# tanmayrainanda/ishara

Measured on AMD Instinct MI355X. Metric: landmark-frames/sec training (B=256,T=384,d=256), higher is better.
Workload: dtype bf16; 1 GPU; configs[1]: get_model(dim=256, 2 squeeze + 2 conformer blocks, kernel_sizes=[11,5,3]) CTC train step (fwd+CTC+bwd+RAdam/Lookahead, dropout on); batch_per_gpu=256, global_batch=256, frames=384, features=224, params=7577784, parallelism=dp1, ranks_seen=1

## Files before the change

ishara_amd/csrc/gemm_as.hip:

```cpp
#include <cstdio>
#include <map>
#include <string>
#include <type_traits>
#include "common.h"
#include "kernels.h"

#ifdef AS_F16
typedef f16 as_t;
typedef f16x8 as_v8;
#define AS_MFMA(b, a, acc) __builtin_amdgcn_mfma_f32_16x16x32_f16(b, a, acc, 0, 0, 0)
#define AS_DT DT_F16
#define AS_NAME(x) x##_f16
#else
typedef bf16 as_t;
typedef bf16x8 as_v8;
#define AS_MFMA(b, a, acc) __builtin_amdgcn_mfma_f32_16x16x32_bf16(b, a, acc, 0, 0, 0)
#define AS_DT DT_BF16
#define AS_NAME(x) x
#endif

extern int g_force_regstage;
bool gemm_nt_as_applicable(int dtC, int M, int N, int K, int ldb, const EpiArgs& ea);

#define AS_NS 32
#define AS_SMALL_M 1536
#define AS_MID_M_K512 32768
#define AS_MAXN 1024

typedef __attribute__((ext_vector_type(4))) uint32_t as_u32x4;

template <int N> DEVI void as_wait_vm() { asm volatile("s_waitcnt vmcnt(%0)" ::"n"(N) : "memory"); }

DEVI int as_swz(int r) { return (r & 3) | (((r >> 3) & 1) << 2); }

template <int GW, typename T> DEVI void as_st(T* p, const float (&v)[GW]) {
    if constexpr (GW == 8) store8(p, v); else store4(p, v);
}
template <int GW, typename T> DEVI void as_st_nt(T* p, const float (&v)[GW], bool nt = true) {
    if constexpr (GW == 8 && is_16b_t<T>::value) {
        as_v8 t;
#pragma unroll
        for (int i = 0; i < 8; ++i) t[i] = (as_t)v[i];
        if (nt) __builtin_nontemporal_store(t, reinterpret_cast<as_v8*>(p)); else *reinterpret_cast<as_v8*>(p) = t;
    } else as_st<GW>(p, v);
}
DEVI void as_st_pk(as_t* p, const as_v8& t, bool nt) {
    if (nt) __builtin_nontemporal_store(t, reinterpret_cast<as_v8*>(p)); else *reinterpret_cast<as_v8*>(p) = t;
}
template <typename TC, int GW> DEVI void as_unpack(const as_u32x4& r, float (&v)[GW]) {
    if constexpr (GW == 8 && std::is_same<TC, f16>::value) {
        const f16x8 h = __builtin_bit_cast(f16x8, r);
#pragma unroll
        for (int e = 0; e < 8; ++e) v[e] = (float)h[e];
    } else if constexpr (GW == 8) {
#pragma unroll
        for (int h = 0; h < 4; ++h) { v[2 * h] = __uint_as_float(r[h] << 16); v[2 * h + 1] = __uint_as_float(r[h] & 0xffff0000u); }
    } else {
#pragma unroll
        for (int h = 0; h < 4; ++h) v[h] = __uint_as_float(r[h]);
    }
}

enum { AS_RESID = 1, AS_DACT = 2, AS_ACT = 4, AS_DROP = 8, AS_ROWSCALE = 16, AS_PREOUT = 32, AS_QKV = 64, AS_ADDTAB = 128, AS_ALL = 255 };
template <int MASK, int F> DEVI bool as_on(bool runtime) {
    if constexpr ((MASK & F) == 0) return false;
    else if constexpr (MASK == AS_ALL) return runtime;
    else return true;
}

template <typename TC, int KT, int MASK, int RT, int DBG, int PRO, int NW = 4, int CS = 1>
DEVI void as_pass(const as_t* __restrict__ A, const as_t* __restrict__ Bt, TC* __restrict__ C, int M, int N, int ldb, const EpiArgs& ea,
                  char* smem, const float* bias_s, int m_base) {
    constexpr int RB = KT * 64;
    constexpr int NS = AS_NS;
    constexpr int SUB = NS * RB;
    constexpr int STAGE = SUB * CS;
    constexpr int R = CS > 1 ? 2 : (KT <= 8 ? 3 : 2);
    constexpr int K = KT * 32;
    constexpr int NI = STAGE / 1024;
    constexpr int DPW = (NI + NW - 1) / NW;
    constexpr bool PAIR = is_16b_t<TC>::value;
    constexpr int GW = PAIR ? 8 : 4;
    constexpr int NG = NS / (4 * GW);
    constexpr int SPS = RT * NG;
    constexpr bool COUNTED = (MASK & (AS_RESID | AS_DACT | AS_ADDTAB | AS_QKV)) == 0;
    constexpr int OPS = SPS * ((MASK & AS_PREOUT) ? 2 : 1);
    constexpr bool HOLDABLE = PAIR && std::is_same<TC, as_t>::value && MASK != AS_ALL && (MASK & AS_QKV) == 0;
    const bool hold = HOLDABLE && (ea.as_flags & 1) && !ea.n_valid;
    const bool nt_side = (ea.as_flags & 2) != 0;

    const int dbg = DBG ? ea.dbg : 0;
    const int tid = threadIdx.x, lane = tid & 63;
    const int wid = __builtin_amdgcn_readfirstlane(tid >> 6);
    const int c = lane & 15, g = lane >> 4;
    const int mw = m_base + wid * 16 * RT;
    const bool full = m_base + NW * 16 * RT <= M;
    const int nsteps = N / NS / (int)gridDim.y;
    const int nbase = (int)blockIdx.y * nsteps * NS;
    const int dmodel = ea.H * ea.dh;
    const bool f_resid = as_on<MASK, AS_RESID>(ea.resid != nullptr), f_dact = as_on<MASK, AS_DACT>(ea.dact != DACT_NONE);
    const bool f_act = as_on<MASK, AS_ACT>(ea.act != ACT_NONE), f_drop = as_on<MASK, AS_DROP>(ea.drop.thr != 0);
    const bool f_rowscale = as_on<MASK, AS_ROWSCALE>(ea.rowscale != nullptr), f_preout = as_on<MASK, AS_PREOUT>(ea.pre_out != nullptr);
    const bool f_qkv = as_on<MASK, AS_QKV>(ea.mode == EPI_QKV), f_addtab = as_on<MASK, AS_ADDTAB>(ea.addtab != nullptr);

    const as_t* bsrc[DPW];
#pragma unroll
    for (int t = 0; t < DPW; ++t) {
        const int o = ((wid * DPW + t) % NI) * 1024 + lane * 16;
        const int r = o / RB, p = (o % RB) >> 4;
        bsrc[t] = Bt + (size_t)(nbase + r) * ldb + ((p ^ as_swz(r)) << 3);
    }
    const size_t bstep = (size_t)NS * CS * ldb;
    auto issue = [&](int slot) {
#pragma unroll
        for (int t = 0; t < DPW; ++t) {
            __builtin_amdgcn_global_load_lds((const __attribute__((address_space(1))) void*)bsrc[t],
                                             (__attribute__((address_space(3))) void*)(smem + slot + ((wid * DPW + t) % NI) * 1024), 16, 0, 0);
            bsrc[t] += bstep;
        }
    };
    const int nstages = (nsteps + CS - 1) / CS;
#pragma unroll
    for (int st = 0; st < R - 1; ++st)
        if (st < nstages && !(dbg & 8)) issue(st * STAGE);

    as_v8 a[RT][KT];
    int mrow[RT];
#pragma unroll
    for (int i = 0; i < RT; ++i) {
        mrow[i] = min(mw + 16 * i + c, M - 1);
        const as_v8* p = reinterpret_cast<const as_v8*>(A + (size_t)mrow[i] * K + g * 8);
#pragma unroll
        for (int kt = 0; kt < KT; ++kt) a[i][kt] = p[kt * 4];
    }

    if constexpr (PRO != 0) {
        float* cs = reinterpret_cast<float*>(smem + (R - 1) * STAGE);
        const int bsm = min(m_base, M - 1) / ea.T;
        const float* c0 = PRO == 1 ? ea.ln_gamma : ea.pa_P + (size_t)bsm * K;
        const float* c1 = PRO == 1 ? ea.ln_beta : ea.pa_Q + (size_t)bsm * K;
        for (int x = tid; x < K; x += NW * 64) { cs[x] = c0[x]; cs[K + x] = c1[x]; }
        __syncthreads();
        auto unpack = [&](const as_v8& f, float (&v)[8]) {
            as_u32x4 t = __builtin_bit_cast(as_u32x4, f);
            asm volatile("" : "+v"(t));
            as_unpack<as_t, 8>(t, v);
        };
        float mean[RT], rstd[RT];
#pragma unroll
        for (int i = 0; i < RT; ++i) { mean[i] = 0.f; rstd[i] = 1.f; }
        if constexpr (PRO == 1) {
#pragma unroll
            for (int i = 0; i < RT; ++i) {
                float s = 0.f;
#pragma unroll
                for (int kt = 0; kt < KT; ++kt) {
                    float v[8];
                    unpack(a[i][kt], v);
#pragma unroll
                    for (int e = 0; e < 8; ++e) s += v[e];
                }
                s += __shfl_xor(s, 16, 64); s += __shfl_xor(s, 32, 64);
                mean[i] = s * (1.f / K);
                float q = 0.f;
#pragma unroll
                for (int kt = 0; kt < KT; ++kt) {
                    float v[8];
                    unpack(a[i][kt], v);
#pragma unroll
                    for (int e = 0; e < 8; ++e) { const float dlt = v[e] - mean[i]; q += dlt * dlt; }
                }
                q += __shfl_xor(q, 16, 64); q += __shfl_xor(q, 32, 64);
                rstd[i] = rsqrtf(q * (1.f / K) + ea.ln_eps);
                const int m = mw + 16 * i + c;
                if (g == 0 && m < M && ea.ln_mean && blockIdx.y == 0) { ea.ln_mean[m] = mean[i]; ea.ln_rstd[m] = rstd[i]; }
            }
        }
#pragma unroll
        for (int kt = 0; kt < KT; ++kt) {
            float wv[8], bv[8];
            {
                const float* cp = cs + 32 * kt + 8 * g;
                asm volatile("" : "+v"(cp));
                const f32x4 w0 = *reinterpret_cast<const f32x4*>(cp), w1 = *reinterpret_cast<const f32x4*>(cp + 4);
                const f32x4 b0 = *reinterpret_cast<const f32x4*>(cp + K), b1 = *reinterpret_cast<const f32x4*>(cp + K + 4);
#pragma unroll
                for (int e = 0; e < 4; ++e) { wv[e] = w0[e]; wv[4 + e] = w1[e]; bv[e] = b0[e]; bv[4 + e] = b1[e]; }
            }
#pragma unroll
            for (int i = 0; i < RT; ++i) {
                float v[8];
                unpack(a[i][kt], v);
                as_v8 t;
#pragma unroll
                for (int e = 0; e < 8; ++e) t[e] = (as_t)(PRO == 1 ? (v[e] - mean[i]) * rstd[i] * wv[e] + bv[e] : v[e] * wv[e] + bv[e]);
                a[i][kt] = t;
            }
        }
        __syncthreads();
    }

    const int frow = PAIR ? 8 * (c >> 2) + (c & 3) : c;
    const int sx = g ^ as_swz(frow);
    const int off_e = frow * RB + ((sx & 3) << 4) + ((sx >> 2) << 6);
    const int off_o = frow * RB + ((sx & 3) << 4) + (((sx >> 2) ^ 1) << 6);
    constexpr int JSTRIDE = (PAIR ? 4 : 16) * RB;

    float rsc[RT];
    uint32_t rk[RT];
    int bsamp[RT];
#pragma unroll
    for (int i = 0; i < RT; ++i) {
        const int m = mw + 16 * i + c;
        rsc[i] = 1.f; rk[i] = 0u; bsamp[i] = 0;
        if (f_rowscale || f_qkv) bsamp[i] = mrow[i] / ea.T;
        if (f_rowscale) rsc[i] = ea.rowscale[bsamp[i]];
        if (f_drop) rk[i] = rng_row_key(ea.drop.key, (uint32_t)m);
    }

    size_t eoff[RT];
#pragma unroll
    for (int i = 0; i < RT; ++i) eoff[i] = (size_t)mrow[i] * (ea.ldc ? ea.ldc : N) + GW * g;
    const TC* resid = reinterpret_cast<const TC*>(ea.resid);
    const TC* aux = reinterpret_cast<const TC*>(ea.aux);

#pragma unroll
    for (int i = 0; i < RT; ++i) {
#pragma unroll
        for (int kt = 0; kt < KT; ++kt) {
            as_u32x4 t = __builtin_bit_cast(as_u32x4, a[i][kt]);
            asm volatile("" : "+v"(t));
            a[i][kt] = __builtin_bit_cast(as_v8, t);
        }
        asm volatile("" : "+v"(rsc[i]));
    }

    as_v8 held[RT], held_pre[RT];
#pragma unroll
    for (int i = 0; i < RT; ++i) { held[i] = as_v8{}; held_pre[i] = as_v8{}; }
    int slot = 0;
    for (int s = 0; s < nsteps; ++s) {
        const int sub = CS > 1 ? (s & (CS - 1)) : 0;
        const bool sync = CS == 1 || sub == 0;
        const int sg = CS > 1 ? s / CS : s;
        if (sync) {
            if constexpr (CS > 1) {
                constexpr bool CCOUNT = MASK != AS_ALL && (MASK & AS_QKV) == 0;
                if (CCOUNT && full && !ea.n_valid && sg >= 1) as_wait_vm<CS * OPS>(); else as_wait_vm<0>();
            } else if constexpr (COUNTED) {
                if (full && !ea.n_valid && s >= R - 1 && s + R - 2 < nsteps) {
                    if (!hold) as_wait_vm<(R - 2) * DPW + (R - 1) * OPS>();
                    else if constexpr (R == 3) as_wait_vm<DPW + 2 * OPS>();
                    else { if (s & 1) as_wait_vm<0>(); else as_wait_vm<2 * OPS>(); }
                } else as_wait_vm<0>();
            } else {
                if (s + R - 2 < nsteps) as_wait_vm<(R - 2) * DPW>(); else as_wait_vm<0>();
            }
            asm volatile("s_waitcnt lgkmcnt(0)" ::: "memory");
            __builtin_amdgcn_s_barrier();
        }
        const int n0 = nbase + s * NS;
        as_u32x4 rs[RT][NG], au[RT][NG];
        if (f_resid) {
#pragma unroll
            for (int i = 0; i < RT; ++i)
#pragma unroll
                for (int q = 0; q < NG; ++q) rs[i][q] = *reinterpret_cast<const as_u32x4*>(resid + eoff[i] + n0 + 4 * GW * q);
        }
        if (f_dact) {
#pragma unroll
            for (int i = 0; i < RT; ++i)
#pragma unroll
                for (int q = 0; q < NG; ++q) au[i][q] = __builtin_nontemporal_load(reinterpret_cast<const as_u32x4*>(aux + eoff[i] + n0 + 4 * GW * q));
        }
        if (sync && sg + R - 1 < nstages && !(dbg & 8)) issue(slot == 0 ? (R - 1) * STAGE : slot - STAGE);
        f32x4 acc[2][RT];
#pragma unroll
        for (int j = 0; j < 2; ++j)
#pragma unroll
            for (int i = 0; i < RT; ++i) acc[j][i] = f32x4{0.f, 0.f, 0.f, 0.f};
        const char* st = smem + slot + sub * SUB;
        if (!(dbg & 6)) {
#pragma unroll
            for (int kt = 0; kt < KT; ++kt) {
#pragma unroll
                for (int j = 0; j < 2; ++j) {
                    const as_v8 b = *reinterpret_cast<const as_v8*>(st + ((kt & 1) ? off_o : off_e) + (kt >> 1) * 128 + j * JSTRIDE);
#pragma unroll
                    for (int i = 0; i < RT; ++i) acc[j][i] = AS_MFMA(b, a[i][kt], acc[j][i]);
                }
            }
        } else if (!(dbg & 4)) {
#pragma unroll
            for (int kt = 0; kt < KT; ++kt)
#pragma unroll
                for (int j = 0; j < 2; ++j) {
                    const f32x4 b = *reinterpret_cast<const f32x4*>(st + ((kt & 1) ? off_o : off_e) + (kt >> 1) * 128 + j * JSTRIDE);
                    acc[j][0] += b;
                }
        } else if (!(dbg & 2)) {
            const as_v8 b = a[0][0];
#pragma unroll
            for (int kt = 0; kt < KT; ++kt)
#pragma unroll
                for (int j = 0; j < 2; ++j)
#pragma unroll
                    for (int i = 0; i < RT; ++i) acc[j][i] = AS_MFMA(b, a[i][kt], acc[j][i]);
        } else {
#pragma unroll
            for (int i = 0; i < RT; ++i) acc[0][i][0] = (float)a[i][0][0] + (float)a[i][KT - 1][7];
        }
        if (dbg & 1) { if (acc[0][0][0] == 123.456f) C[0] = from_f<TC>(acc[1][RT - 1][2]); if (CS == 1 || sub == CS - 1) slot = slot == (R - 1) * STAGE ? 0 : slot + STAGE; continue; }
#pragma unroll
        for (int q = 0; q < NG; ++q) {
            const int n = n0 + 4 * GW * q + GW * g;
            if (ea.n_valid && n >= ea.n_valid) continue;
            float bias[GW];
#pragma unroll
            for (int h = 0; h < GW / 4; ++h) {
                const f32x4 bv = *reinterpret_cast<const f32x4*>(bias_s + n + 4 * h);
#pragma unroll
                for (int e = 0; e < 4; ++e) bias[4 * h + e] = bv[e];
            }
#pragma unroll
            for (int i = 0; i < RT; ++i) {
                const int m = mw + 16 * i + c;
                if (!full && m >= M) continue;
                const size_t off = eoff[i] + n0 + 4 * GW * q;
                float v[GW];
                const float bsc = (f_rowscale && ea.rowscale_bias) ? rsc[i] : 1.f;
                if constexpr (PAIR) {
#pragma unroll
                    for (int e = 0; e < 4; ++e) { v[e] = acc[0][i][e] + bias[e] * bsc; v[4 + e] = acc[1][i][e] + bias[4 + e] * bsc; }
                } else {
#pragma unroll
                    for (int e = 0; e < 4; ++e) v[e] = acc[q][i][e] + bias[e] * bsc;
                }
                if (f_addtab) {
                    const float* tp = ea.addtab + (size_t)(m % ea.tab_period) * N + n;
#pragma unroll
                    for (int h = 0; h < GW / 4; ++h) {
                        float t4[4];
                        load4(tp + 4 * h, t4);
#pragma unroll
                        for (int e = 0; e < 4; ++e) v[4 * h + e] += t4[e];
                    }
                }
                if (f_preout) {
                    if constexpr (HOLDABLE) {
                        if (hold) {
                            as_v8 t;
#pragma unroll
                            for (int e = 0; e < 8; ++e) t[e] = (as_t)v[e];
                            as_t* pp = reinterpret_cast<as_t*>(ea.pre_out) + off;
                            if (s & 1) { as_st_pk(pp - NS, held_pre[i], nt_side); as_st_pk(pp, t, nt_side); }
                            else if (s == nsteps - 1) as_st_pk(pp, t, nt_side);
                            else held_pre[i] = t;
                        } else as_st_nt<GW>(reinterpret_cast<TC*>(ea.pre_out) + off, v, nt_side);
                    } else as_st_nt<GW>(reinterpret_cast<TC*>(ea.pre_out) + off, v, nt_side);
                }
                if (f_act) {
                    if (ea.act == ACT_SWISH) {
#pragma unroll
                        for (int e = 0; e < GW; ++e) v[e] = swishf_(v[e]);
                    } else {
#pragma unroll
                        for (int e = 0; e < GW; ++e) v[e] = fmaxf(v[e], 0.f);
                    }
                }
                if (f_drop) {
                    rng_apply<GW>(rk[i], (uint32_t)n, ea.drop.thr, ea.drop.scale, v);
                }
                if (f_rowscale && !ea.rowscale_bias) {
#pragma unroll
                    for (int e = 0; e < GW; ++e) v[e] *= rsc[i];
                }
                if (f_dact) {
                    float x[GW];
                    as_unpack<TC, GW>(au[i][q], x);
                    if (ea.dact == DACT_SWISH) {
#pragma unroll
                        for (int e = 0; e < GW; ++e) v[e] *= dswishf_(x[e]);
                    } else {
#pragma unroll
                        for (int e = 0; e < GW; ++e) v[e] = x[e] > 0.f ? v[e] : 0.f;
                    }
                }
                if (f_resid) {
                    float x[GW];
                    as_unpack<TC, GW>(rs[i][q], x);
#pragma unroll
                    for (int e = 0; e < GW; ++e) v[e] += x[e];
                }
                if (!f_qkv) {
                    if constexpr (HOLDABLE) {
                        if (hold) {
                            as_v8 t;
#pragma unroll
                            for (int e = 0; e < 8; ++e) t[e] = (as_t)v[e];
                            as_t* cp = reinterpret_cast<as_t*>(C) + off;
                            if (s & 1) { as_st_pk(cp - NS, held[i], false); as_st_pk(cp, t, false); }
                            else if (s == nsteps - 1) as_st_pk(cp, t, false);
                            else held[i] = t;
                        } else as_st<GW>(C + off, v);
                    } else as_st<GW>(C + off, v);
                } else {
                    int h, part, ii;
                    if (ea.head_major) { h = n / (3 * ea.dh); const int w = n - h * 3 * ea.dh; part = w / ea.dh; ii = w - part * ea.dh; }
                    else { part = n / dmodel; const int w = n - part * dmodel; h = w / ea.dh; ii = w - h * ea.dh; }
                    const int t = m - bsamp[i] * ea.T;
                    if (part < 2) {
                        as_st<GW>(reinterpret_cast<TC*>(part == 0 ? ea.q : ea.k) + ((size_t)(bsamp[i] * ea.H + h) * ea.T + t) * ea.dh + ii, v);
                    } else {
                        TC* dst = reinterpret_cast<TC*>(ea.vt) + ((size_t)(bsamp[i] * ea.H + h) * ea.dh + ii) * ea.T + t;
#pragma unroll
                        for (int e = 0; e < GW; ++e) dst[(size_t)e * ea.T] = from_f<TC>(v[e]);
                    }
                }
            }
        }
        if (CS == 1 || sub == CS - 1) slot = slot == (R - 1) * STAGE ? 0 : slot + STAGE;
    }
    if constexpr (PRO != 0) {
        if (ea.pro_out && blockIdx.y == 0) {
#pragma unroll
            for (int i = 0; i < RT; ++i) {
                const int m = mw + 16 * i + c;
                if (m < M) {
                    as_v8* p = reinterpret_cast<as_v8*>(reinterpret_cast<as_t*>(ea.pro_out) + (size_t)m * K + g * 8);
#pragma unroll
                    for (int kt = 0; kt < KT; ++kt) as_st_pk(reinterpret_cast<as_t*>(&p[kt * 4]), a[i][kt], nt_side);
                }
            }
        }
    }
}

template <typename TC, int KT, int MASK, int DBG = 0, int PRO = 0>
__global__ __launch_bounds__(KT <= 16 ? 256 : 512, KT <= 8 ? 3 : (KT <= 16 ? 2 : 1)) void gemm_nt_as_kernel(const as_t* __restrict__ A, const as_t* __restrict__ Bt, TC* __restrict__ C,
                                                                         int M, int N, int ldb, EpiArgs ea) {
    constexpr int R = KT <= 8 ? 3 : 2;
    constexpr int STAGE = AS_NS * KT * 64;
    __shared__ __attribute__((aligned(16))) char smem[R * STAGE + AS_MAXN * 4];
    float* bias_s = reinterpret_cast<float*>(smem + R * STAGE);
    for (int n = threadIdx.x; n < N; n += (int)blockDim.x) bias_s[n] = (ea.bias && (!ea.n_valid || n < ea.n_valid)) ? ea.bias[n] : 0.f;
    if constexpr (KT <= 8) {
        if (M <= AS_SMALL_M) as_pass<TC, KT, MASK, 1, DBG, PRO>(A, Bt, C, M, N, ldb, ea, smem, bias_s, blockIdx.x * 64);
        else as_pass<TC, KT, MASK, 2, DBG, PRO>(A, Bt, C, M, N, ldb, ea, smem, bias_s, blockIdx.x * 128);
    } else if constexpr (KT >= 32) {
        as_pass<TC, KT, MASK, 1, DBG, PRO, 8>(A, Bt, C, M, N, ldb, ea, smem, bias_s, blockIdx.x * 128);
    } else if (M <= AS_MID_M_K512) {
        as_pass<TC, KT, MASK, 1, DBG, PRO>(A, Bt, C, M, N, ldb, ea, smem, bias_s, blockIdx.x * 64);
    } else {
        const int m_base = blockIdx.x * 192;
        as_pass<TC, KT, MASK, 2, DBG, PRO>(A, Bt, C, M, N, ldb, ea, smem, bias_s, m_base);
        if (m_base + 128 < M) {
            __builtin_amdgcn_s_barrier();
            as_pass<TC, KT, MASK, 1, DBG, PRO>(A, Bt, C, M, N, ldb, ea, smem, bias_s, m_base + 128);
        }
    }
}

#define AS_CHUNK_ROWS 384
template <int KT> struct AsChunk { static constexpr int NW = KT <= 8 ? 12 : 8, CS = KT <= 8 ? 4 : 2; };
template <typename TC, int KT, int MASK, int PRO = 0>
__global__ __launch_bounds__(AsChunk<KT>::NW * 64, 1) void gemm_nt_as_chunk_kernel(const as_t* __restrict__ A, const as_t* __restrict__ Bt, TC* __restrict__ C, int M, int N, int ldb, EpiArgs ea) {
    extern __shared__ __attribute__((aligned(16))) char csm[];
    constexpr int NW = AsChunk<KT>::NW, CS = AsChunk<KT>::CS;
    constexpr int STAGE = AS_NS * KT * 64 * CS;
    float* bias_s = reinterpret_cast<float*>(csm + 2 * STAGE);
    for (int n = threadIdx.x; n < N; n += (int)blockDim.x) bias_s[n] = (ea.bias && (!ea.n_valid || n < ea.n_valid)) ? ea.bias[n] : 0.f;
    const int m_base = blockIdx.x * AS_CHUNK_ROWS;
    if constexpr (KT <= 8) {
        as_pass<TC, KT, MASK, 2, 0, PRO, NW, CS>(A, Bt, C, M, N, ldb, ea, csm, bias_s, m_base);
    } else {
        as_pass<TC, KT, MASK, 2, 0, PRO, NW, CS>(A, Bt, C, M, N, ldb, ea, csm, bias_s, m_base);
        if (m_base + 256 < M) {
            __builtin_amdgcn_s_barrier();
            as_pass<TC, KT, MASK, 1, 0, PRO, NW, CS>(A, Bt, C, M, N, ldb, ea, csm, bias_s, m_base + 256);
        }
    }
}
template <typename KF> static bool as_chunk_prepare(KF kernel, int bytes) {
    static std::map<const void*, bool> done;
    const void* key = reinterpret_cast<const void*>(kernel);
    auto it = done.find(key);
    if (it != done.end()) return it->second;
    const bool ok = hipFuncSetAttribute(key, hipFuncAttributeMaxDynamicSharedMemorySize, bytes) == hipSuccess;
    done[key] = ok;
    return ok;
}

static int as_mask_of(const EpiArgs& ea) {
    return (ea.resid ? AS_RESID : 0) | (ea.dact != DACT_NONE ? AS_DACT : 0) | (ea.act != ACT_NONE ? AS_ACT : 0) | (ea.drop.thr ? AS_DROP : 0) |
           (ea.rowscale ? AS_ROWSCALE : 0) | (ea.pre_out ? AS_PREOUT : 0) | (ea.mode == EPI_QKV ? AS_QKV : 0) | (ea.addtab ? AS_ADDTAB : 0);
}

static int as_inst_mask(bool c_bf16, int mask, int K = 256) {
    if (!c_bf16) return mask == 0 ? 0 : AS_ALL;
    if (K == 128) return (mask == AS_DACT || mask == (AS_DACT | AS_DROP)) ? mask : AS_ALL;
    switch (mask) {
        case 0: case AS_RESID: case AS_RESID | AS_ROWSCALE: case AS_ROWSCALE: case AS_RESID | AS_DROP: case AS_ACT | AS_PREOUT: case AS_ACT | AS_PREOUT | AS_DROP:
        case AS_ACT | AS_DROP: case AS_ACT: case AS_DACT: case AS_DACT | AS_DROP: case AS_QKV: case AS_ADDTAB: return mask;
        default: return AS_ALL;
    }
}

#define AS_LAUNCH_PLAIN(MASK, PRO) hipLaunchKernelGGL((gemm_nt_as_kernel<TC, KT, MASK, 0, PRO>), grid, block, 0, s, (const as_t*)A, (const as_t*)Bt, (TC*)C, M, N, ldb, ea)
#ifdef AS_F16
#define AS_LAUNCH2(MASK, PRO) AS_LAUNCH_PLAIN(MASK, PRO)
#else
#define AS_LAUNCH2(MASK, PRO)                                                                                                         \
    do {                                                                                                                              \
        if constexpr ((KT == 8 || KT == 16) && std::is_same<TC, as_t>::value && (MASK) != AS_ALL) {                                   \
            constexpr int CB = 2 * AS_NS * KT * 64 * AsChunk<KT>::CS + AS_MAXN * 4;                                                   \
            if (chunked && as_chunk_prepare(gemm_nt_as_chunk_kernel<TC, KT, MASK, PRO>, CB)) {                                        \
                hipLaunchKernelGGL((gemm_nt_as_chunk_kernel<TC, KT, MASK, PRO>), dim3((M + AS_CHUNK_ROWS - 1) / AS_CHUNK_ROWS), dim3(AsChunk<KT>::NW * 64), CB, s, \
                                   (const as_t*)A, (const as_t*)Bt, (TC*)C, M, N, ldb, ea);                                           \
                break;                                                                                                                \
            }                                                                                                                         \
        }                                                                                                                             \
        AS_LAUNCH_PLAIN(MASK, PRO);                                                                                                   \
    } while (0)
#endif
#define AS_LAUNCH(MASK) AS_LAUNCH2(MASK, 0)
#ifdef AS_F16
extern int g_as_flags_override;
#else
int g_as_flags_override = -1;
#endif
static int as_default_flags() {
    static const int v = getenv("ISHARA_AS_FLAGS") ? atoi(getenv("ISHARA_AS_FLAGS")) : 51;
    return g_as_flags_override >= 0 ? g_as_flags_override : v;
}
static bool as_chunk_applies(int flags, int M, int N, int K, const EpiArgs& ea) {
    const int cs = K == 256 ? 4 : 2;
    return (K == 256 ? (flags & 16) : (K == 512 && (flags & 32))) && M >= 128 * AS_CHUNK_ROWS && (N / AS_NS) % cs == 0 && N >= 128 && !ea.n_valid && !ea.dbg &&
           (!ea.pa_P || (ea.T > 0 && ea.T % AS_CHUNK_ROWS == 0));
}
template <typename TC, int KT>
static int run_as(const void* A, const void* Bt, void* C, int M, int N, int ldb, const EpiArgs& ea_in, hipStream_t s) {
    EpiArgs ea = ea_in;
    if (ea.as_flags < 0) ea.as_flags = as_default_flags();
    const int BR = KT <= 8 ? (M <= AS_SMALL_M ? 64 : 128) : (KT <= 16 ? (M <= AS_MID_M_K512 ? 64 : 192) : 128);
    const int gx = (M + BR - 1) / BR, slots = KT <= 8 ? 768 : (KT <= 16 ? 512 : 256);
    int gy = 1;
    const int max_gy = M <= AS_SMALL_M ? 16 : 4, min_cols = M <= AS_SMALL_M ? 32 : 128;
    while (gy < max_gy && gx * gy * 2 <= slots && (N / AS_NS) % (gy * 2) == 0 && N / (gy * 2) >= min_cols) gy *= 2;
    const dim3 grid(gx, gy), block(KT <= 16 ? 256 : 512);
    const int mask = as_mask_of(ea);
    const bool chunked = (KT == 8 || KT == 16) && as_chunk_applies(ea.as_flags, M, N, KT * 32, ea) && gy == 1;
    (void)chunked;
    if constexpr (is_16b_t<TC>::value && KT >= 8) {
#define AS_PRO(MASK, PRO) AS_LAUNCH2(MASK, PRO)
        if (ea.ln_gamma) {
            switch (mask) {
                case 0: AS_PRO(0, 1); break;
                case AS_ACT | AS_PREOUT: AS_PRO(AS_ACT | AS_PREOUT, 1); break;
                case AS_ACT | AS_PREOUT | AS_DROP: AS_PRO(AS_ACT | AS_PREOUT | AS_DROP, 1); break;
                case AS_QKV: AS_PRO(AS_QKV, 1); break;
                default: ishara_set_error("gemm_nt_as: LayerNorm prologue with epilogue mask %d is not compiled", mask); return -1;
            }
            return hipGetLastError() == hipSuccess ? 0 : -2;
        }
        if (ea.pa_P) {
            switch (mask) {
                case AS_RESID: AS_PRO(AS_RESID, 2); break;
                case AS_RESID | AS_ROWSCALE: AS_PRO(AS_RESID | AS_ROWSCALE, 2); break;
                default: ishara_set_error("gemm_nt_as: affine prologue with epilogue mask %d is not compiled", mask); return -1;
            }
            return hipGetLastError() == hipSuccess ? 0 : -2;
        }
#undef AS_PRO
    }
    if constexpr (KT == 4) {
        if (mask == AS_DACT) AS_LAUNCH(AS_DACT); else if (mask == (AS_DACT | AS_DROP)) AS_LAUNCH(AS_DACT | AS_DROP); else AS_LAUNCH(AS_ALL);
    }
#ifdef AS_F16
    else if constexpr (is_16b_t<TC>::value) {
        switch (mask) {
            case 0: AS_LAUNCH(0); break;
            case AS_RESID: AS_LAUNCH(AS_RESID); break;
            case AS_ACT | AS_PREOUT: AS_LAUNCH(AS_ACT | AS_PREOUT); break;
            case AS_ACT: AS_LAUNCH(AS_ACT); break;
            case AS_QKV: AS_LAUNCH(AS_QKV); break;
            case AS_ADDTAB: AS_LAUNCH(AS_ADDTAB); break;
            default: AS_LAUNCH(AS_ALL); break;
        }
    }
#else
    else if constexpr (is_16b_t<TC>::value) {
        switch (mask) {
            case 0:
                if (ea.dbg) hipLaunchKernelGGL((gemm_nt_as_kernel<TC, KT, 0, 1>), grid, block, 0, s, (const as_t*)A, (const as_t*)Bt, (TC*)C, M, N, ldb, ea);
                else AS_LAUNCH(0);
                break;
            case AS_RESID: AS_LAUNCH(AS_RESID); break;
            case AS_RESID | AS_ROWSCALE: AS_LAUNCH(AS_RESID | AS_ROWSCALE); break;
            case AS_ROWSCALE: AS_LAUNCH(AS_ROWSCALE); break;
            case AS_RESID | AS_DROP: AS_LAUNCH(AS_RESID | AS_DROP); break;
            case AS_ACT | AS_PREOUT: AS_LAUNCH(AS_ACT | AS_PREOUT); break;
            case AS_ACT | AS_PREOUT | AS_DROP: AS_LAUNCH(AS_ACT | AS_PREOUT | AS_DROP); break;
            case AS_ACT | AS_DROP: AS_LAUNCH(AS_ACT | AS_DROP); break;
            case AS_ACT: AS_LAUNCH(AS_ACT); break;
            case AS_DACT: AS_LAUNCH(AS_DACT); break;
            case AS_DACT | AS_DROP: AS_LAUNCH(AS_DACT | AS_DROP); break;
            case AS_QKV: AS_LAUNCH(AS_QKV); break;
            case AS_ADDTAB: AS_LAUNCH(AS_ADDTAB); break;
            default: AS_LAUNCH(AS_ALL); break;
        }
    }
#endif
    else {
        if (mask == 0) AS_LAUNCH(0); else AS_LAUNCH(AS_ALL);
    }
    return hipGetLastError() == hipSuccess ? 0 : -2;
}
#undef AS_LAUNCH

#ifndef AS_F16
bool gemm_nt_as_prologue_ok(int dtA, int dtM, int dtC, int M, int N, int K, int ldb, const EpiArgs& ea) {
    if (!dt_is16(dtA) || dtM != dtA || dtC != dtA || (K != 256 && K != 512 && !(K == 1024 && dtA == DT_BF16)) || !gemm_nt_as_applicable(dtC, M, N, K, ldb, ea)) return false;
    if (ldb % 64 != 0 || g_force_regstage) return false;
    const int BR = K == 256 ? (M <= AS_SMALL_M ? 64 : 128) : (K == 512 ? (M <= AS_MID_M_K512 ? 64 : 192) : 128), gx = (M + BR - 1) / BR, slots = K == 256 ? 768 : (K == 512 ? 512 : 256);
    (void)gx; (void)slots;
    const int mask = as_mask_of(ea);
    if (ea.ln_gamma) return mask == 0 || mask == (AS_ACT | AS_PREOUT) || mask == (AS_ACT | AS_PREOUT | AS_DROP) || mask == AS_QKV;
    if (ea.pa_P) return ea.T > 0 && ea.T % BR == 0 && (mask == AS_RESID || mask == (AS_RESID | AS_ROWSCALE));
    return false;
}

bool gemm_nt_as_applicable(int dtC, int M, int N, int K, int ldb, const EpiArgs& ea) {
    if (K != 256 && K != 512 && !((K == 128 || K == 1024) && dtC == DT_BF16)) return false;
    if (N % AS_NS != 0 || N > AS_MAXN || ldb < K || ldb % 8 != 0 || M < 1) return false;
    if (ea.mode == EPI_QKV && (ea.dh % 8 != 0 || ea.T % 8 != 0)) return false;
    return true;
}

const char* gemm_nt_as_name(int dtC, int K, const EpiArgs& ea, int M, int N) {
    static std::map<int, std::string> names;
    const int inst = as_inst_mask(dtC == DT_BF16, as_mask_of(ea), K);
    const int pro = ea.ln_gamma ? 1 : (ea.pa_P ? 2 : 0);
    const bool chunk = dtC == DT_BF16 && inst != AS_ALL && as_chunk_applies(ea.as_flags < 0 ? as_default_flags() : ea.as_flags, M, N, K, ea);
    const int id = (dtC == DT_BF16 ? 0 : 1 << 20) | (pro << 22) | (chunk ? 1 << 24 : 0) | (K << 8) | inst;
    auto it = names.find(id);
    if (it == names.end()) {
        char buf[96];
        if (chunk) snprintf(buf, sizeof buf, "gemm_nt_as_chunk_kernel<bf16,%d,%d,%d>", K / 32, pro ? as_mask_of(ea) : inst, pro);
        else if (pro) snprintf(buf, sizeof buf, "gemm_nt_as_kernel<%s,%d,%d,0,%d>", dtC == DT_BF16 ? "bf16" : "f32", K / 32, as_mask_of(ea), pro);
        else snprintf(buf, sizeof buf, "gemm_nt_as_kernel<%s,%d,%d,0>", dtC == DT_BF16 ? "bf16" : "f32", K / 32, inst);
        it = names.emplace(id, buf).first;
    }
    return it->second.c_str();
}

#endif

#ifdef AS_F16
int launch_gemm_nt_as_f16(int dtC, const void* A, const void* Bt, void* C, int M, int N, int K, int ldb, const EpiArgs& ea, hipStream_t s) {
    if ((K != 256 && K != 512) || !gemm_nt_as_applicable(dtC, M, N, K, ldb, ea)) return 1;
    if (dtC == DT_F16) return K == 256 ? run_as<f16, 8>(A, Bt, C, M, N, ldb, ea, s) : run_as<f16, 16>(A, Bt, C, M, N, ldb, ea, s);
    return K == 256 ? run_as<float, 8>(A, Bt, C, M, N, ldb, ea, s) : run_as<float, 16>(A, Bt, C, M, N, ldb, ea, s);
}
#else
int launch_gemm_nt_as(int dtC, const void* A, const void* Bt, void* C, int M, int N, int K, int ldb, const EpiArgs& ea, hipStream_t s) {
    if (!gemm_nt_as_applicable(dtC, M, N, K, ldb, ea)) return 1;
    if (dtC == DT_BF16) return K == 128 ? run_as<bf16, 4>(A, Bt, C, M, N, ldb, ea, s) : (K == 256 ? run_as<bf16, 8>(A, Bt, C, M, N, ldb, ea, s) :
                               (K == 512 ? run_as<bf16, 16>(A, Bt, C, M, N, ldb, ea, s) : run_as<bf16, 32>(A, Bt, C, M, N, ldb, ea, s)));
    return K == 256 ? run_as<float, 8>(A, Bt, C, M, N, ldb, ea, s) : run_as<float, 16>(A, Bt, C, M, N, ldb, ea, s);
}
#endif
```

Baseline: 6.818 million frames/s.

## Add pipelined K=512 chunk GEMM path overlapping A prefetch and B DMA

```diff
diff --git a/ishara_amd/csrc/gemm_as.hip b/ishara_amd/csrc/gemm_as.hip
--- a/ishara_amd/csrc/gemm_as.hip
+++ b/ishara_amd/csrc/gemm_as.hip
@@ -463,7 +463,276 @@
 
 #define AS_CHUNK_ROWS 384
 template <int KT> struct AsChunk { static constexpr int NW = KT <= 8 ? 12 : 8, CS = KT <= 8 ? 4 : 2; };
-template <typename TC, int KT, int MASK, int PRO = 0>
+
+#ifndef AS_F16
+DEVI void as_ld_raw(as_u32x4& d, const as_t* p) { asm volatile("global_load_dwordx4 %0, %1, off" : "=&v"(d) : "v"(p)); }
+DEVI void as_ld_raw_nt(as_u32x4& d, const as_t* p) { asm volatile("global_load_dwordx4 %0, %1, off nt" : "=&v"(d) : "v"(p)); }
+DEVI void as_wait_vm_n(int n) {
+    switch (n) {
+#define AS_W(N) case N: as_wait_vm<N>(); break;
+        AS_W(1) AS_W(2) AS_W(3) AS_W(4) AS_W(5) AS_W(6) AS_W(7) AS_W(8) AS_W(9) AS_W(10) AS_W(11) AS_W(12) AS_W(13) AS_W(14) AS_W(15) AS_W(16)
+#undef AS_W
+        default: as_wait_vm<0>(); break;
+    }
+}
+
+template <typename TC, int KT, int MASK, int PRO, int NW, int CS>
+DEVI void as_pipe(const as_t* __restrict__ A, const as_t* __restrict__ Bt, TC* __restrict__ C, int M, int N, int ldb, const EpiArgs& ea,
+                  char* smem, const float* bias_s, const float* cs, int m_base) {
+    static_assert(std::is_same<TC, as_t>::value && MASK != AS_ALL && (MASK & (AS_QKV | AS_ADDTAB)) == 0 && CS % 2 == 0, "as_pipe: 16-bit C, a compiled feature mask, whole store pairs per stage");
+    constexpr int RB = KT * 64, NS = AS_NS, SUB = NS * RB, STAGE = SUB * CS, K = KT * 32;
+    constexpr int NI = STAGE / 1024, DPW = NI / NW;
+    static_assert(NI % NW == 0, "as_pipe: the waves share a stage's DMA evenly");
+    constexpr int SR = NW * 16;
+    constexpr int NP = AS_CHUNK_ROWS / SR;
+    constexpr int OPS = (MASK & AS_PREOUT) ? 2 : 1;
+    constexpr int PFS = 2, PFK = KT / PFS;
+    const bool hold = (ea.as_flags & 1) != 0;
+    const bool nt_side = (ea.as_flags & 2) != 0;
+
+    const int tid = threadIdx.x, lane = tid & 63;
+    const int wid = __builtin_amdgcn_readfirstlane(tid >> 6);
+    const int c = lane & 15, g = lane >> 4;
+    const int nsteps = N / NS, nstages = nsteps / CS;
+    constexpr bool f_resid = (MASK & AS_RESID) != 0, f_dact = (MASK & AS_DACT) != 0, f_act = (MASK & AS_ACT) != 0, f_drop = (MASK & AS_DROP) != 0;
+    constexpr bool f_rowscale = (MASK & AS_ROWSCALE) != 0, f_preout = (MASK & AS_PREOUT) != 0;
+
+    const as_t* bsrc[DPW];
+#pragma unroll
+    for (int t = 0; t < DPW; ++t) {
+        const int o = (wid * DPW + t) * 1024 + lane * 16;
+        const int r = o / RB, p = (o % RB) >> 4;
+        bsrc[t] = Bt + (size_t)r * ldb + ((p ^ as_swz(r)) << 3);
+    }
+    const size_t bstep = (size_t)NS * CS * ldb;
+    auto issue = [&](int slot, int stage) {
+#pragma unroll
+        for (int t = 0; t < DPW; ++t)
+            __builtin_amdgcn_global_load_lds((const __attribute__((address_space(1))) void*)(bsrc[t] + stage * bstep),
+                                             (__attribute__((address_space(3))) void*)(smem + slot + (wid * DPW + t) * 1024), 16, 0, 0);
+    };
+    issue(0, 0);
+
+    auto arow = [&](int p) { return reinterpret_cast<const as_v8*>(A + (size_t)min(m_base + p * SR + wid * 16 + c, M - 1) * K + g * 8); };
+    as_v8 a[2][KT];
+    {
+        const as_v8* p0 = arow(0);
+#pragma unroll
+        for (int kt = 0; kt < KT; ++kt) a[0][kt] = p0[kt * 4];
+    }
+    if constexpr (PRO != 0) __syncthreads();
+
+    const int frow = 8 * (c >> 2) + (c & 3);
+    const int sx = g ^ as_swz(frow);
+    const int off_e = frow * RB + ((sx & 3) << 4) + ((sx >> 2) << 6);
+    const int off_o = frow * RB + ((sx & 3) << 4) + (((sx >> 2) ^ 1) << 6);
+    constexpr int JSTRIDE = 4 * RB;
+    const as_t* resid = reinterpret_cast<const as_t*>(ea.resid);
+    const as_t* aux = reinterpret_cast<const as_t*>(ea.aux);
+
+    int slot = 0;
+    auto subpass = [&](auto PC) {
+        constexpr int P = decltype(PC)::value;
+        as_v8 (&ac)[KT] = a[P & 1];
+        as_v8 (&an)[KT] = a[(P + 1) & 1];
+        const int m = m_base + P * SR + wid * 16 + c, mrow = min(m, M - 1);
+        const bool full = m_base + (P + 1) * SR <= M;
+        const bool has_next = P + 1 < NP && m_base + (P + 1) * SR < M;
+        const as_v8* pn = arow(P + 1);
+
+#pragma unroll
+        for (int kt = 0; kt < KT; ++kt) {
+            as_u32x4 t = __builtin_bit_cast(as_u32x4, ac[kt]);
+            asm volatile("" : "+v"(t));
+            ac[kt] = __builtin_bit_cast(as_v8, t);
+        }
+        float mean = 0.f, rstd = 1.f;
+        if constexpr (PRO != 0) {
+            auto unpack = [&](const as_v8& f, float (&v)[8]) {
+                as_u32x4 t = __builtin_bit_cast(as_u32x4, f);
+                asm volatile("" : "+v"(t));
+                as_unpack<as_t, 8>(t, v);
+            };
+            if constexpr (PRO == 1) {
+                float s = 0.f;
+#pragma unroll
+                for (int kt = 0; kt < KT; ++kt) {
+                    float v[8];
+                    unpack(ac[kt], v);
+#pragma unroll
+                    for (int e = 0; e < 8; ++e) s += v[e];
+                }
+                s += __shfl_xor(s, 16, 64); s += __shfl_xor(s, 32, 64);
+                mean = s * (1.f / K);
+                float q = 0.f;
+#pragma unroll
+                for (int kt = 0; kt < KT; ++kt) {
+                    float v[8];
+                    unpack(ac[kt], v);
+#pragma unroll
+                    for (int e = 0; e < 8; ++e) { const float dlt = v[e] - mean; q += dlt * dlt; }
+                }
+                q += __shfl_xor(q, 16, 64); q += __shfl_xor(q, 32, 64);
+                rstd = rsqrtf(q * (1.f / K) + ea.ln_eps);
+            }
+#pragma unroll
+            for (int kt = 0; kt < KT; ++kt) {
+                int co = 32 * kt + 8 * g;
+                if (kt >= 2) {
+                    as_u32x4 d = __builtin_bit_cast(as_u32x4, ac[kt - 2]);
+                    asm volatile("" : "+v"(co), "+v"(d));
+                    ac[kt - 2] = __builtin_bit_cast(as_v8, d);
+                } else asm volatile("" : "+v"(co));
+                const float* cp = cs + co;
+                const f32x4 w0 = *reinterpret_cast<const f32x4*>(cp), w1 = *reinterpret_cast<const f32x4*>(cp + 4);
+                const f32x4 b0 = *reinterpret_cast<const f32x4*>(cp + K), b1 = *reinterpret_cast<const f32x4*>(cp + K + 4);
+                float wv[8], bv[8], v[8];
+#pragma unroll
+                for (int e = 0; e < 4; ++e) { wv[e] = w0[e]; wv[4 + e] = w1[e]; bv[e] = b0[e]; bv[4 + e] = b1[e]; }
+                unpack(ac[kt], v);
+                as_v8 t;
+#pragma unroll
+                for (int e = 0; e < 8; ++e) t[e] = (as_t)(PRO == 1 ? (v[e] - mean) * rstd * wv[e] + bv[e] : v[e] * wv[e] + bv[e]);
+                ac[kt] = t;
+            }
+        }
+
+        float rsc = 1.f;
+        uint32_t rk = 0u;
+        if constexpr (f_rowscale) rsc = ea.rowscale[mrow / ea.T];
+        if constexpr (f_drop) rk = rng_row_key(ea.drop.key, (uint32_t)m);
+        const size_t eoff = (size_t)mrow * (ea.ldc ? ea.ldc : N) + 8 * g;
+        asm volatile("" : "+v"(rsc));
+
+        as_v8 held = as_v8{}, held_pre = as_v8{};
+        for (int sg = 0; sg < nstages; ++sg) {
+            if ((P > 0 || sg > 0) && (sg == 0 || full)) as_wait_vm<CS * OPS>(); else as_wait_vm<0>();
+            asm volatile("s_waitcnt lgkmcnt(0)" ::: "memory");
+            __builtin_amdgcn_s_barrier();
+            if (has_next) {
+#pragma unroll
+                for (int h = 0; h < PFS; ++h)
+                    if (sg == h) {
+#pragma unroll
+                        for (int kt = h * PFK; kt < (h + 1) * PFK; ++kt) an[kt] = pn[kt * 4];
+                    }
+            }
+            if constexpr (PRO != 0) {
+                if (ea.pro_out && m < M) {
+                    as_v8* po = reinterpret_cast<as_v8*>(reinterpret_cast<as_t*>(ea.pro_out) + (size_t)m * K + g * 8);
+#pragma unroll
+                    for (int h = 0; h < PFS; ++h)
+                        if (sg == PFS + h) {
+#pragma unroll
+                            for (int kt = h * PFK; kt < (h + 1) * PFK; ++kt) as_st_pk(reinterpret_cast<as_t*>(&po[kt * 4]), ac[kt], nt_side);
+                        }
+                }
+                if (PRO == 1 && sg == PFS && g == 0 && m < M && ea.ln_mean) { ea.ln_mean[m] = mean; ea.ln_rstd[m] = rstd; }
+            }
+            constexpr int NL = (f_resid ? 1 : 0) + (f_dact ? 1 : 0);
+            as_u32x4 rsv[CS], auv[CS];
+#pragma unroll
+            for (int sub = 0; sub < CS; ++sub) {
+                if constexpr (f_resid) as_ld_raw(rsv[sub], resid + eoff + (sg * CS + sub) * NS);
+                if constexpr (f_dact) as_ld_raw_nt(auv[sub], aux + eoff + (sg * CS + sub) * NS);
+            }
+            const bool last = sg + 1 == nstages;
+            const bool dma = !last || has_next;
+            if (dma) issue(slot ^ STAGE, last ? 0 : sg + 1);
+#pragma unroll
+            for (int sub = 0; sub < CS; ++sub) {
+                const int n0 = (sg * CS + sub) * NS;
+                f32x4 acc[2] = {f32x4{0.f, 0.f, 0.f, 0.f}, f32x4{0.f, 0.f, 0.f, 0.f}};
+                const char* st = smem + slot + sub * SUB;
+#pragma unroll
+                for (int kt = 0; kt < KT; ++kt) {
+#pragma unroll
+                    for (int j = 0; j < 2; ++j) {
+                        const as_v8 b = *reinterpret_cast<const as_v8*>(st + ((kt & 1) ? off_o : off_e) + (kt >> 1) * 128 + j * JSTRIDE);
+                        acc[j] = AS_MFMA(b, ac[kt], acc[j]);
+                    }
+                }
+                const int n = n0 + 8 * g;
+                as_u32x4 rs, au;
+                if constexpr (NL > 0) {
+                    as_wait_vm_n(full ? (CS - 1 - sub) * NL + (dma ? DPW : 0) + (hold ? (sub / 2) * 2 : sub) * OPS : 0);
+                    if constexpr (f_resid) { rs = rsv[sub]; asm volatile("" : "+v"(rs)); }
+                    if constexpr (f_dact) { au = auv[sub]; asm volatile("" : "+v"(au)); }
+                }
+                if (!full && m >= M) continue;
+                float bias[8];
+#pragma unroll
+                for (int h = 0; h < 2; ++h) {
+                    const f32x4 bv = *reinterpret_cast<const f32x4*>(bias_s + n + 4 * h);
+#pragma unroll
+                    for (int e = 0; e < 4; ++e) bias[4 * h + e] = bv[e];
+                }
+                const size_t off = eoff + n0;
+                float v[8];
+                const float bsc = (f_rowscale && ea.rowscale_bias) ? rsc : 1.f;
+#pragma unroll
+                for (int e = 0; e < 4; ++e) { v[e] = acc[0][e] + bias[e] * bsc; v[4 + e] = acc[1][e] + bias[4 + e] * bsc; }
+                if constexpr (f_preout) {
+                    as_t* pp = reinterpret_cast<as_t*>(ea.pre_out) + off;
+                    if (hold) {
+                        as_v8 t;
+#pragma unroll
+                        for (int e = 0; e < 8; ++e) t[e] = (as_t)v[e];
+                        if (sub & 1) { as_st_pk(pp - NS, held_pre, nt_side); as_st_pk(pp, t, nt_side); }
+                        else held_pre = t;
+                    } else as_st_nt<8>(pp, v, nt_side);
+                }
+                if constexpr (f_act) {
+                    if (ea.act == ACT_SWISH) {
+#pragma unroll
+                        for (int e = 0; e < 8; ++e) v[e] = swishf_(v[e]);
+                    } else {
+#pragma unroll
+                        for (int e = 0; e < 8; ++e) v[e] = fmaxf(v[e], 0.f);
+                    }
+                }
+                if constexpr (f_drop) rng_apply<8>(rk, (uint32_t)n, ea.drop.thr, ea.drop.scale, v);
+                if (f_rowscale && !ea.rowscale_bias) {
+#pragma unroll
+                    for (int e = 0; e < 8; ++e) v[e] *= rsc;
+                }
+                if constexpr (f_dact) {
+                    float x[8];
+                    as_unpack<as_t, 8>(au, x);
+                    if (ea.dact == DACT_SWISH) {
+#pragma unroll
+                        for (int e = 0; e < 8; ++e) v[e] *= dswishf_(x[e]);
+                    } else {
+#pragma unroll
+                        for (int e = 0; e < 8; ++e) v[e] = x[e] > 0.f ? v[e] : 0.f;
+                    }
+                }
+                if constexpr (f_resid) {
+                    float x[8];
+                    as_unpack<as_t, 8>(rs, x);
+#pragma unroll
+                    for (int e = 0; e < 8; ++e) v[e] += x[e];
+                }
+                as_t* cp = reinterpret_cast<as_t*>(C) + off;
+                if (hold) {
+                    as_v8 t;
+#pragma unroll
+                    for (int e = 0; e < 8; ++e) t[e] = (as_t)v[e];
+                    if (sub & 1) { as_st_pk(cp - NS, held, false); as_st_pk(cp, t, false); }
+                    else held = t;
+                } else as_st<8>(cp, v);
+            }
+            slot ^= STAGE;
+        }
+    };
+    subpass(std::integral_constant<int, 0>{});
+    if (m_base + SR < M) subpass(std::integral_constant<int, 1>{});
+    if constexpr (NP > 2) { if (m_base + 2 * SR < M) subpass(std::integral_constant<int, 2>{}); }
+    static_assert(NP == 2 || NP == 3, "as_pipe: two or three sub-passes");
+}
+#endif
+
+template <typename TC, int KT, int MASK, int PRO = 0, int PIPE = 0>
 __global__ __launch_bounds__(AsChunk<KT>::NW * 64, 1) void gemm_nt_as_chunk_kernel(const as_t* __restrict__ A, const as_t* __restrict__ Bt, TC* __restrict__ C, int M, int N, int ldb, EpiArgs ea) {
     extern __shared__ __attribute__((aligned(16))) char csm[];
     constexpr int NW = AsChunk<KT>::NW, CS = AsChunk<KT>::CS;
@@ -471,6 +740,20 @@
     float* bias_s = reinterpret_cast<float*>(csm + 2 * STAGE);
     for (int n = threadIdx.x; n < N; n += (int)blockDim.x) bias_s[n] = (ea.bias && (!ea.n_valid || n < ea.n_valid)) ? ea.bias[n] : 0.f;
     const int m_base = blockIdx.x * AS_CHUNK_ROWS;
+#ifndef AS_F16
+    if constexpr (PIPE != 0) {
+        float* cs = bias_s + AS_MAXN;
+        if constexpr (PRO != 0) {
+            constexpr int K = KT * 32;
+            const int bsm = PRO == 2 ? min(m_base, M - 1) / ea.T : 0;
+            const float* c0 = PRO == 1 ? ea.ln_gamma : ea.pa_P + (size_t)bsm * K;
+            const float* c1 = PRO == 1 ? ea.ln_beta : ea.pa_Q + (size_t)bsm * K;
+            for (int x = threadIdx.x; x < K; x += NW * 64) { cs[x] = c0[x]; cs[K + x] = c1[x]; }
+        }
+        as_pipe<TC, KT, MASK, PRO, NW, CS>(A, Bt, C, M, N, ldb, ea, csm, bias_s, cs, m_base);
+        return;
+    }
+#endif
     if constexpr (KT <= 8) {
         as_pass<TC, KT, MASK, 2, 0, PRO, NW, CS>(A, Bt, C, M, N, ldb, ea, csm, bias_s, m_base);
     } else {
@@ -512,6 +795,14 @@
 #else
 #define AS_LAUNCH2(MASK, PRO)                                                                                                         \
     do {                                                                                                                              \
+        if constexpr (KT == 16 && std::is_same<TC, as_t>::value && (MASK) != AS_ALL && ((MASK) & (AS_QKV | AS_ADDTAB)) == 0) {        \
+            constexpr int PB = 2 * AS_NS * KT * 64 * AsChunk<KT>::CS + AS_MAXN * 4 + 2 * KT * 32 * 4;                                 \
+            if (chunked && as_pipe_applies(ea.as_flags, N, KT * 32) && as_chunk_prepare(gemm_nt_as_chunk_kernel<TC, KT, MASK, PRO, 1>, PB)) { \
+                hipLaunchKernelGGL((gemm_nt_as_chunk_kernel<TC, KT, MASK, PRO, 1>), dim3((M + AS_CHUNK_ROWS - 1) / AS_CHUNK_ROWS), dim3(AsChunk<KT>::NW * 64), PB, s, \
+                                   (const as_t*)A, (const as_t*)Bt, (TC*)C, M, N, ldb, ea);                                           \
+                break;                                                                                                                \
+            }                                                                                                                         \
+        }                                                                                                                             \
         if constexpr ((KT == 8 || KT == 16) && std::is_same<TC, as_t>::value && (MASK) != AS_ALL) {                                   \
             constexpr int CB = 2 * AS_NS * KT * 64 * AsChunk<KT>::CS + AS_MAXN * 4;                                                   \
             if (chunked && as_chunk_prepare(gemm_nt_as_chunk_kernel<TC, KT, MASK, PRO>, CB)) {                                        \
@@ -524,13 +815,14 @@
     } while (0)
 #endif
 #define AS_LAUNCH(MASK) AS_LAUNCH2(MASK, 0)
+static bool as_pipe_applies(int flags, int N, int K) { return K == 512 && (flags & 64) && N >= 4 * AS_NS * AsChunk<16>::CS; }
 #ifdef AS_F16
 extern int g_as_flags_override;
 #else
 int g_as_flags_override = -1;
 #endif
 static int as_default_flags() {
-    static const int v = getenv("ISHARA_AS_FLAGS") ? atoi(getenv("ISHARA_AS_FLAGS")) : 51;
+    static const int v = getenv("ISHARA_AS_FLAGS") ? atoi(getenv("ISHARA_AS_FLAGS")) : 115;
     return g_as_flags_override >= 0 ? g_as_flags_override : v;
 }
 static bool as_chunk_applies(int flags, int M, int N, int K, const EpiArgs& ea) {
@@ -642,11 +934,13 @@
     const int inst = as_inst_mask(dtC == DT_BF16, as_mask_of(ea), K);
     const int pro = ea.ln_gamma ? 1 : (ea.pa_P ? 2 : 0);
     const bool chunk = dtC == DT_BF16 && inst != AS_ALL && as_chunk_applies(ea.as_flags < 0 ? as_default_flags() : ea.as_flags, M, N, K, ea);
-    const int id = (dtC == DT_BF16 ? 0 : 1 << 20) | (pro << 22) | (chunk ? 1 << 24 : 0) | (K << 8) | inst;
+    const bool pipe = chunk && (inst & (AS_QKV | AS_ADDTAB)) == 0 && as_pipe_applies(ea.as_flags < 0 ? as_default_flags() : ea.as_flags, N, K);
+    const int id = (dtC == DT_BF16 ? 0 : 1 << 20) | (pro << 22) | (chunk ? 1 << 24 : 0) | (pipe ? 1 << 25 : 0) | (K << 8) | inst;
     auto it = names.find(id);
     if (it == names.end()) {
         char buf[96];
-        if (chunk) snprintf(buf, sizeof buf, "gemm_nt_as_chunk_kernel<bf16,%d,%d,%d>", K / 32, pro ? as_mask_of(ea) : inst, pro);
+        if (pipe) snprintf(buf, sizeof buf, "gemm_nt_as_chunk_kernel<bf16,%d,%d,%d,1>", K / 32, pro ? as_mask_of(ea) : inst, pro);
+        else if (chunk) snprintf(buf, sizeof buf, "gemm_nt_as_chunk_kernel<bf16,%d,%d,%d>", K / 32, pro ? as_mask_of(ea) : inst, pro);
         else if (pro) snprintf(buf, sizeof buf, "gemm_nt_as_kernel<%s,%d,%d,0,%d>", dtC == DT_BF16 ? "bf16" : "f32", K / 32, as_mask_of(ea), pro);
         else snprintf(buf, sizeof buf, "gemm_nt_as_kernel<%s,%d,%d,0>", dtC == DT_BF16 ? "bf16" : "f32", K / 32, inst);
         it = names.emplace(id, buf).first;
```

Result: no change. 6.751 million frames/s (-1.0%).
